# dwkim606/optimal_conv

Measured on AMD Instinct MI355X. Metric: homomorphic convs/sec (conv_then_pack + BN bias, k x k, batch B, N=2^16), higher is better.
Workload: dtype u64; 1 GPU; conv 3 3; ker_wid=3, batch=256, in_wid=16, logN=16, moduli=ckks.DefaultBootstrapParams[6] Q0,Q1 + P=0x1fffffffffe00001, ciphertexts_per_launch_set=4, contexts_per_gpu=4, chunk_nodes=512

## Files before the change

optimal_conv_amd/csrc/hc_arith.h:

```cpp
#pragma once
#include <stdint.h>

#if defined(__HIPCC__) || defined(HC_EMU)
#define HC_HD __host__ __device__ __forceinline__
#else
#define HC_HD inline
#endif

typedef uint64_t u64;
typedef unsigned int u32;
typedef unsigned __int128 u128;

HC_HD u64 hc_mulhi(u64 a, u64 b) {
#if defined(__HIP_DEVICE_COMPILE__)
    return __umul64hi(a, b);
#else
    return (u64)(((u128)a * b) >> 64);
#endif
}

HC_HD u64 hc_mul_shoup_lazy(u64 x, u64 w, u64 wp, u64 q) {
    u64 hi = hc_mulhi(x, wp);
    return x * w - hi * q;
}
HC_HD double hc_f64_mulmod(double x, double w, double wq, double q) {
#pragma clang fp contract(off)
    const double h = x * w;
    const double l = __builtin_fma(x, w, -h);
    const double k = __builtin_rint(x * wq);
    const double r = __builtin_fma(-k, q, h);
    return r + l;
}
HC_HD double hc_f64_reduce(double u, double q, double qinv) {
#pragma clang fp contract(off)
    return __builtin_fma(-__builtin_rint(u * qinv), q, u);
}
HC_HD double hc_u2d(u64 x) { return __builtin_bit_cast(double, x); }
HC_HD u64 hc_d2u(double x) { return __builtin_bit_cast(u64, x); }
HC_HD double hc_f64_from_u(u64 x) { return hc_u2d(x | 0x4330000000000000ull) - 4503599627370496.0; }
HC_HD u64 hc_f64_to_u_plus(double v, u64 base) { return (hc_d2u(v + 6755399441055744.0) & 0x000FFFFFFFFFFFFFull) + (base - 0x0008000000000000ull); }

HC_HD u64 hc_shoup_companion(u64 w, u64 q) {
    u64 r = w, quo = 0;
    for (int i = 0; i < 64; i++) {
        r <<= 1; quo <<= 1;
        if (r >= q) { r -= q; quo |= 1; }
    }
    return quo;
}
HC_HD u64 hc_csub(u64 x, u64 q) { return x >= q ? x - q : x; }

HC_HD u64 hc_mulhi_lo2(u64 x, u64 p) {
    const u32 x0 = (u32)x, x1 = (u32)(x >> 32), p0 = (u32)p, p1 = (u32)(p >> 32);
    return (u64)x1 * p1 + (((u64)x0 * p1) >> 32) + (((u64)x1 * p0) >> 32);
}
HC_HD u64 hc_opaque_uniform(u64 v) {
#if defined(__HIP_DEVICE_COMPILE__)
    u64 r;
    asm("; uniform constant kept opaque" : "=s"(r) : "0"(v));
    return r;
#else
    return v;
// ... 43 lines not shown
```

optimal_conv_amd/csrc/hc_kernels.h:

```cpp
#pragma once
#include "hc_arith.h"

#define HC_TPB 256
#ifndef HC_MIN_WAVES
#define HC_MIN_WAVES 4
#endif
#define HC_ROWS_LDS 4096
#define HC_COLS_LDS 4096

struct __attribute__((aligned(16))) HcTw { u64 w, ws; };

#define HC_SMALL_Q(q) ((q) < (1ull << 31))
template <bool B> struct HcBool { static constexpr bool value = B; };
template <int V> struct HcInt { static constexpr int value = V; };
#define HC_COUNT_DISPATCH(n, body) do { switch (n) { case 1: body(HcInt<1>{}); break; case 2: body(HcInt<2>{}); break; case 3: body(HcInt<3>{}); break; case 4: body(HcInt<4>{}); break; \
    case 5: body(HcInt<5>{}); break; case 6: body(HcInt<6>{}); break; case 7: body(HcInt<7>{}); break; case 8: body(HcInt<8>{}); break; default: break; } } while (0)
#define HC_LD(S32, rowptr, j) ((S32) ? hc_ld32(rowptr, j) : (rowptr)[j])
#define HC_ST(S32, rowptr, j, v) do { if (S32) hc_st32(rowptr, j, v); else (rowptr)[j] = (v); } while (0)
#define HC_ROW_DISPATCH(row32, body) do { if (row32) body(HcBool<true>{}); else body(HcBool<false>{}); } while (0)
__device__ __forceinline__ u64 hc_ld32(const u64 *row, size_t j) { return (u64)reinterpret_cast<const u32 *>(row)[j]; }
__device__ __forceinline__ void hc_st32(u64 *row, size_t j, u64 v) { reinterpret_cast<u32 *>(row)[j] = (u32)v; }
struct __attribute__((packed, aligned(4))) HcU64A4 { u64 v; };
__device__ __forceinline__ u64 hc_ldp(const u64 *row, size_t j, bool row32) {
    return reinterpret_cast<const HcU64A4 *>(reinterpret_cast<const char *>(row) + (j << (row32 ? 2 : 3)))->v & (row32 ? 0xFFFFFFFFull : ~0ull);
// ... 618 lines not shown
        const u64 x = t[i];
        u64 r;
        if (x > (q0 >> 1)) { r = hc_barrett64(q0 - x, q, mu); r = r ? q - r : 0; }
        else r = hc_barrett64(x, q, mu);
        if (row32) hc_st32(out, i, r); else out[i] = r;
    }
}
__global__ __launch_bounds__(HC_TPB) void hc_k_shoup_companion(const u64 *w, u64 *ws, size_t n, u64 q) {
    for (size_t i = (size_t)blockIdx.x * HC_TPB + threadIdx.x; i < n; i += (size_t)gridDim.x * HC_TPB)
        ws[i] = hc_shoup_companion(w[i], q);
}
__global__ __launch_bounds__(HC_TPB) void hc_k_lo_local(const u64 *in, u64 *out, size_t n) {
    for (size_t i = (size_t)blockIdx.x * HC_TPB + threadIdx.x; i < n; i += (size_t)gridDim.x * HC_TPB) {
        const size_t poly = i >> 16; const int R = (int)((i >> 8) & 255), C = (int)(i & 255);
        out[(poly << 16) + (size_t)(((R >> 4) * 16 + (C & 15)) * 256 + (R & 15) * 16 + (C >> 4))] = in[i];
    }
}
__global__ __launch_bounds__(HC_TPB) void hc_k_make_pairs(const u64 *w, HcTw *out, size_t n, u64 q, int lo_local_order) {
    for (size_t i = (size_t)blockIdx.x * HC_TPB + threadIdx.x; i < n; i += (size_t)gridDim.x * HC_TPB) {
        u64 x = w[i];
        HcTw p; p.w = x; p.ws = hc_shoup_companion(x, q);
        size_t j = i;
        if (lo_local_order) {
            size_t poly = i >> 16; int R = (int)((i >> 8) & 255), C = (int)(i & 255);
            j = (poly << 16) + (size_t)(((R >> 4) * 16 + (C & 15)) * 256 + (R & 15) * 16 + (C >> 4));
        }
        out[j] = p;
    }
}

#define HC_MAXB 16
struct HcPtrs { const u64 *p[HC_MAXB]; };
struct HcCtc { HcMod m0, m1; HcTw c0, c1; };
__global__ __launch_bounds__(HC_TPB) void hc_k_ctc_pairs(HcPtrs ct_in, HcTw *out, HcCtc K) {
    const int r = blockIdx.y, l = r & 1; const HcMod m = l ? K.m1 : K.m0; const HcTw cst = l ? K.c1 : K.c0;
    const u64 *in = ct_in.p[blockIdx.z] + (size_t)r * 65536;
    HcTw *o = out + ((size_t)blockIdx.z * 4 + r) * 65536;
    for (size_t i = (size_t)blockIdx.x * HC_TPB + threadIdx.x; i < 65536; i += (size_t)gridDim.x * HC_TPB) {
        HcTw p; p.w = hc_mul_shoup(in[i], cst.w, cst.ws, m.q); p.ws = hc_shoup_companion(p.w, m.q);
        o[i] = p;
    }
}

struct HcPrepKer {
    const double *ker_in;
    const double *bn_a;
    u64 *stage;
    int in_wid, ker_wid, real_ib, real_ob, norm, max_bat;
    double scale;
    u64 q0, q1;
    int src_wid, dil, ib_stride;
};
__device__ __forceinline__ void hc_prep_ker_put(const HcPrepKer &P, int k_sz, int vec_size, int adj, int i, int col, double v) {
    const int jj = P.max_bat - 1 - col / k_sz, kk = k_sz - 1 - col % k_sz;
    const int p0 = (P.in_wid * (kk / P.ker_wid) + kk % P.ker_wid) * P.max_bat + jj;
    const bool wrap = p0 < adj;
    const int p = wrap ? vec_size - adj + p0 : p0 - adj;
    const double val = wrap ? -v : v;
    const bool neg = val < 0;
    const double x = neg ? -P.scale * val : P.scale * val;
    const u64 xi = (u64)(x + 0.5);
    const u64 r0 = xi % P.q0, r1 = xi % P.q1;
    P.stage[((size_t)0 * P.max_bat + i) * 65536 + p] = neg ? P.q0 - r0 : r0;
    P.stage[((size_t)1 * P.max_bat + i) * 65536 + p] = neg ? P.q1 - r1 : r1;
}
template <bool TRANS, bool EXP = false, bool FC = false>
__global__ __launch_bounds__(HC_TPB) void hc_k_prep_ker(HcPrepKer P) {
    static_assert(!(TRANS && EXP), "dilated / channel-strided kernels have no transposed form");
    static_assert(!FC || EXP, "the shared-matrix form is a form of the dilated scatter");
// ... 73 lines not shown
#ifndef HC_W_A3
#define HC_W_A3 3
#endif
#ifndef HC_W_B1
#define HC_W_B1 4
#endif
#ifndef HC_W_B2
#define HC_W_B2 1
#endif
#ifndef HC_W_B3
#define HC_W_B3 4
#endif
#ifndef HC_W_B4
#define HC_W_B4 1
#endif
#ifndef HC_A3_ROWS
#define HC_A3_ROWS 4
#endif
struct HcLoopA {
    const HcTw *ctc;
    HcPtrs ker;
    u64 *tmp;
    u64 *cts;
    int i0, norm;
    int slot0, slot_step;
    size_t cts_stride;
    int njobs;
    int gm;
    HcMod m0, m1;
    HcTw q1inv;
    u64 h, negh0;
};
template <int F64>
__global__ __launch_bounds__(HC_TPB, HC_W_A1) void hc_k_a1p(HcLoopA A, HcTwTab T1inv) {
    __shared__ __attribute__((aligned(16))) u64 lds[HC_ROWS_LDS];
    const int t = threadIdx.x, tid = t & 15, rloc = t >> 4, row = HC_TILE * 16 + rloc;
    const int ch = HC_JOB, i = A.i0 + ch * A.norm, z = blockIdx.z;
    const HcTw *__restrict__ c0 = A.ctc + ((size_t)z * 4 + 1) * 65536 + (size_t)HC_TILE * 4096 + t;
    const u64 *__restrict__ k = A.ker.p[z] + ((size_t)i * 2 + 1) * 65536 + (size_t)HC_TILE * 4096 + t;
    const HcQ Q = hc_q(A.m1.q);
    const HcTw wA = hc_twl_load(T1inv, HC_TILE, t);
    u64 e0[16], e1[16];
#pragma unroll
    for (int kk = 0; kk < 16; kk++) {
        const u64 kv = k[kk * 256];
        const HcTw w0 = c0[kk * 256], w1 = c0[2 * 65536 + kk * 256];
        e0[kk] = hc_shoup4(kv, w0.w, w0.ws, Q);
        e1[kk] = hc_shoup4(kv, w1.w, w1.ws, Q);
    }
    u64 *o = A.tmp + ((size_t)z * A.njobs + 2 * ch) * 65536 + (size_t)row * 256;
    hc_xchg(lds, [&](int kk) { return hc_rows_lds(kk, t); }, [&](int lo) { return hc_rows_lds(rloc, tid * 16 + lo); }, [] { __syncthreads(); }, e0, e1);
    HC_ROW_SYNC();
    if (F64) {
        const HcF64Mod m{(double)A.m1.q, 1.0 / (double)A.m1.q};
        double f0[16], f1[16];
#pragma unroll
        for (int kk = 0; kk < 16; kk++) { f0[kk] = hc_f64_reduce(hc_f64_from_u(e0[kk]), m.q, m.qinv); f1[kk] = hc_f64_reduce(hc_f64_from_u(e1[kk]), m.q, m.qinv); }
        hc_rows_inv2_f64(f0, f1, lds, T1inv, wA, row, rloc, tid, m);
#pragma unroll
        for (int hi = 0; hi < 16; hi++) { o[hi * 16 + tid] = hc_d2u(f0[hi]); o[65536 + hi * 16 + tid] = hc_d2u(f1[hi]); }
    } else {
        hc_rows_inv_twl(HcLazy<>{Q}, lds, T1inv, wA, row, rloc, tid, e0, e1);
#pragma unroll
        for (int hi = 0; hi < 16; hi++) { o[hi * 16 + tid] = e0[hi]; o[65536 + hi * 16 + tid] = e1[hi]; }
    }
}
__device__ __forceinline__ void hc_rows_inv2_f64_g(double (&f0)[16], double (&f1)[16], u64 *lds, const HcTwTab &T, const HcTw &wA, int row, int rloc, int tid, HcF64Mod m) {
    hc_gs_round2_f64(f0, f1, HcTwB<false, HcTw>{T.rowsB + row * 256 + tid}, m);
    u64 b0[16], b1[16];
#pragma unroll
    for (int i = 0; i < 16; i++) { b0[i] = hc_d2u(f0[i]); b1[i] = hc_d2u(f1[i]); }
    hc_xchg(lds, [&](int lo) { return hc_rows_lds(rloc, tid * 16 + lo); }, [&](int hi) { return hc_rows_lds(rloc, hi * 16 + tid); }, [] { HC_ROW_SYNC(); }, b0, b1);
#pragma unroll
    for (int i = 0; i < 16; i++) { f0[i] = hc_u2d(b0[i]); f1[i] = hc_u2d(b1[i]); }
    hc_gs_round2_f64(f0, f1, hc_twl_put(lds, wA, rloc, tid), m);
}
template <int FM>
__device__ __forceinline__ void hc_rows_fwd2_lin_g(u64 (&e0)[16], u64 (&e1)[16], u64 *lds, const HcTwTab &T, const HcTw &wA, int row, int rloc, int tid, int t, const HcQ &Q) {
    hc_ct_round(HcLazy<FM>{Q}, hc_twl_put(lds, wA, rloc, tid), e0, e1);
    HC_ROW_SYNC();
    hc_xchg(lds, [&](int hi) { return hc_rows_lds(rloc, hi * 16 + tid); }, [&](int lo) { return hc_rows_lds(rloc, tid * 16 + lo); }, [] { HC_ROW_SYNC(); }, e0, e1);
    hc_ct_round(HcLazy<FM>{Q}, HcTwB<false, HcTw>{T.rowsB + row * 256 + tid}, e0, e1);
    HC_ROW_SYNC();
    hc_xchg(lds, [&](int lo) { return hc_rows_lds(rloc, tid * 16 + lo); }, [&](int kk) { return hc_rows_lds(kk, t); }, [] { __syncthreads(); }, e0, e1);
}
template <int F64>
__global__ __launch_bounds__(HC_TPB, HC_W_A1) void hc_k_a1g(HcLoopA A, HcTwTab T1inv) {
    __shared__ __attribute__((aligned(16))) u64 lds[HC_ROWS_LDS];
    const int t = threadIdx.x, tid = t & 15, rloc = t >> 4, row = HC_TILE * 16 + rloc;
    const int ch = HC_JOB, i = A.i0 + ch * A.norm, g = blockIdx.z, m = A.gm;
    const size_t tile = (size_t)HC_TILE * 4096 + t;
    const HcQ Q = hc_q(A.m1.q);
    const HcTw wA = hc_twl_load(T1inv, HC_TILE, t);
    const HcF64Mod fm{(double)A.m1.q, 1.0 / (double)A.m1.q};
    u64 e0[16], e1[16];
    if (F64) {
        double f0[16], f1[16];
#pragma unroll
        for (int kk = 0; kk < 16; kk++) f0[kk] = f1[kk] = 0.0;
        for (int j = 0; j < m; j += 2) {
            const bool two = j + 1 < m;
            const int za = g * m + j, zb = two ? za + 1 : za;
            const HcTw *__restrict__ ca = A.ctc + ((size_t)za * 4 + 1) * 65536 + tile, *__restrict__ cb = A.ctc + ((size_t)zb * 4 + 1) * 65536 + tile;
            const u64 *__restrict__ ka = A.ker.p[za] + ((size_t)i * 2 + 1) * 65536 + tile, *__restrict__ kb = A.ker.p[zb] + ((size_t)i * 2 + 1) * 65536 + tile;
#pragma unroll
            for (int kk = 0; kk < 16; kk++) {
                const u64 kv = ka[kk * 256];
                const HcTw w0 = ca[kk * 256], w1 = ca[2 * 65536 + kk * 256];
                u64 s0 = hc_shoup4(kv, w0.w, w0.ws, Q), s1 = hc_shoup4(kv, w1.w, w1.ws, Q);
                if (two) {
                    const u64 kv2 = kb[kk * 256];
                    const HcTw x0 = cb[kk * 256], x1 = cb[2 * 65536 + kk * 256];
                    s0 += hc_shoup4(kv2, x0.w, x0.ws, Q); s1 += hc_shoup4(kv2, x1.w, x1.ws, Q);
                }
                f0[kk] += hc_f64_reduce(hc_f64_from_u(s0), fm.q, fm.qinv); f1[kk] += hc_f64_reduce(hc_f64_from_u(s1), fm.q, fm.qinv);
            }
        }
#pragma unroll
        for (int kk = 0; kk < 16; kk++) { e0[kk] = hc_d2u(hc_f64_reduce(f0[kk], fm.q, fm.qinv)); e1[kk] = hc_d2u(hc_f64_reduce(f1[kk], fm.q, fm.qinv)); }
    } else {
#pragma unroll
        for (int kk = 0; kk < 16; kk++) e0[kk] = e1[kk] = 0;
        for (int j = 0; j < m; j++) {
            const int z = g * m + j;
            const HcTw *__restrict__ c0 = A.ctc + ((size_t)z * 4 + 1) * 65536 + tile;
            const u64 *__restrict__ k = A.ker.p[z] + ((size_t)i * 2 + 1) * 65536 + tile;
#pragma unroll
            for (int kk = 0; kk < 16; kk++) {
                const u64 kv = k[kk * 256];
                const HcTw w0 = c0[kk * 256], w1 = c0[2 * 65536 + kk * 256];
                e0[kk] = hc_fold(e0[kk] + hc_canon4(hc_shoup4(kv, w0.w, w0.ws, Q), Q), Q.nq);
                e1[kk] = hc_fold(e1[kk] + hc_canon4(hc_shoup4(kv, w1.w, w1.ws, Q), Q), Q.nq);
            }
        }
    }
    u64 *o = A.tmp + ((size_t)g * A.njobs + 2 * ch) * 65536 + (size_t)row * 256;
    hc_xchg(lds, [&](int kk) { return hc_rows_lds(kk, t); }, [&](int lo) { return hc_rows_lds(rloc, tid * 16 + lo); }, [] { __syncthreads(); }, e0, e1);
    HC_ROW_SYNC();
    if (F64) {
        double f0[16], f1[16];
#pragma unroll
        for (int kk = 0; kk < 16; kk++) { f0[kk] = hc_u2d(e0[kk]); f1[kk] = hc_u2d(e1[kk]); }
        hc_rows_inv2_f64_g(f0, f1, lds, T1inv, wA, row, rloc, tid, fm);
#pragma unroll
        for (int hi = 0; hi < 16; hi++) { o[hi * 16 + tid] = hc_d2u(f0[hi]); o[65536 + hi * 16 + tid] = hc_d2u(f1[hi]); }
    } else {
        hc_rows_inv_twl(HcLazy<>{Q}, lds, T1inv, wA, row, rloc, tid, e0, e1);
#pragma unroll
        for (int hi = 0; hi < 16; hi++) { o[hi * 16 + tid] = e0[hi]; o[65536 + hi * 16 + tid] = e1[hi]; }
    }
}
template <int FM, int F64>
// ... 2002 lines not shown
```

optimal_conv_amd/csrc/hconv.hip:

```cpp
#ifdef HC_EMU
#include "hip_emu.h"
#else
#include <hip/hip_runtime.h>
#endif

#include <math.h>
#include <stdarg.h>
#include <stdio.h>
#include <string.h>

#include <atomic>
#include <map>
#include <utility>
#include <string>
#include <vector>

#include "../../include/hconv.h"
#include "../../include/hconv_test_hooks.h"
#include "hc_kernels.h"
#include "hc_gomath.h"
#ifndef HC_GX_LV
#define HC_GX_LV 64
#endif
#ifndef HC_GX_PW
// ... 51 lines not shown
    if (n > 1) fac.push_back(n);
    for (u64 g = 3;; g++) {
        bool ok = true;
        for (u64 f : fac) if (h_powmod(g, (q - 1) / f, q) == 1) { ok = false; break; }
        if (ok) return g;
    }
}
static u32 h_bitrev16(u32 x) { u32 r = 0; for (int i = 0; i < 16; i++) { r = (r << 1) | (x & 1); x >>= 1; } return r; }

struct HcModHost {
    HcMod m;
    u64 psi, psi_inv;
    HcTwTab fwd, inv;
    HcTwTab32 fwd32 = {nullptr, nullptr, nullptr, nullptr}, inv32 = {nullptr, nullptr, nullptr, nullptr};
    HcTwTab inv_f64;
    std::vector<void *> allocs;
};
struct HcEvk { HcTw *q_rows; HcTw *p_rows; u64 *q_mont; bool row_local; bool row256; };
struct HcSwk { u64 *rows = nullptr; int level = 0, beta = 0; };
struct HcProfRec { std::string name; hipEvent_t a, b; };
struct hc_ctx {
    int device = 0, nq = 0, np = 0;
    hipStream_t stream = nullptr;
    std::vector<HcModHost> mods;
    std::map<u64, HcEvk> evk;
    std::map<u64, HcSwk> swk;
    HcTw *idx_pairs = nullptr;
    u64 *idx_mont = nullptr;
    bool idx_mono = false;
    u64 idx_gen = 0;
    u64 *ws_cts = nullptr; size_t ws_cts_rows = 0;
    u64 *ws_cts2 = nullptr; size_t ws_cts2_rows = 0;
    HcTw *ws_ctc = nullptr; size_t ws_ctc_cts = 0;
    u64 *ws_tmp = nullptr; size_t ws_tmp_rows = 0;
    HcMod *d_mods = nullptr; HcTw *d_csts = nullptr;
    u64 *d_mono = nullptr;
    struct CacheBlk { size_t n = 0; hipEvent_t ev = nullptr; bool pending = false; };
    std::map<char *, CacheBlk> cache_blk; std::map<size_t, std::vector<void *>> cache_free;
    int async_alloc = 0;
#ifdef HC_EMU
    long small_mm_wgs = 0;
#else
    long small_mm_wgs = 1024;
#endif
    long allocs_live = 0;
    std::map<const char *, size_t> user_blk;
    HcRowMod *d_rowmods = nullptr;
    u64 *ws_mm = nullptr; size_t ws_mm_rows = 0;
    u64 *ws_accm = nullptr; size_t ws_accm_rows = 0;
    struct KsPlan { HcBasisExt *bx = nullptr, *bxdown = nullptr; HcTw *pinv = nullptr, *pmod = nullptr, *pinv_qlinv = nullptr, *yinv = nullptr, *yinv1 = nullptr; };
    std::map<int, KsPlan> ks_plan;
    std::map<int, HcTw *> rescale_plan;
    int nb = 1; size_t bs_poly = 0, bs_qp = 0;
    const void *hoist_cx = nullptr; int hoist_level = -1;
    long chunk_nodes = 64;
    hipEvent_t ev_fork = nullptr;
    HcCplx *enc_roots = nullptr; int *enc_rot_group = nullptr;
    u32 *d_flag = nullptr;
    u64 *crt_tab = nullptr; std::vector<int> crt_words;
    hipEvent_t ev_shard = nullptr;
    u64 *ws_gather = nullptr; size_t ws_gather_rows = 0;
    long small_levels = 16;
    long peer_access = 1;
    int xcd_rows = 1;
    int pack32 = 1;
    int rot_fuse = 1;
// ... 210 lines not shown
        std::vector<u64> mono(c->mods.size() * HC_MONO_WORDS);
        for (size_t i = 0; i < c->mods.size(); i++) {
            const u64 qi = c->mods[i].m.q, r = (u64)((((u128)1) << 64) % qi), psi256 = h_powmod(c->mods[i].psi, HC_MONO_LO, qi);
            u64 *t = &mono[i * HC_MONO_WORDS], w = r;
            for (int k = 0; k < HC_MONO_LO; k++) { t[k] = w; w = h_mulmod(w, c->mods[i].psi, qi); }
            w = r;
            for (int k = 0; k < HC_MONO_HI; k++) { t[HC_MONO_LO + k] = w; w = h_mulmod(w, psi256, qi); }
        }
        if (hcx_malloc(c, (void **)&c->d_mono, mono.size() * sizeof(u64)) != hipSuccess || hcx_h2d(c, c->d_mono, mono.data(), mono.size() * sizeof(u64)) != hipSuccess) {
            g_create_err = "hc_ctx_create: device table of psi powers"; hc_ctx_destroy(c); return HC_ERR_HIP; }
    }
    if (hcx_malloc(c, (void **)&c->d_rowmods, c->mods.size() * sizeof(HcRowMod)) != hipSuccess || hc_upload_rowmods(c) != HC_OK) { g_create_err = "hc_ctx_create: device table of transforms"; hc_ctx_destroy(c); return HC_ERR_HIP; }
    *out = c;
    return HC_OK;
}

extern "C" void hc_ctx_destroy(hc_ctx *c) {
    if (!c) return;
    hipError_t first = hipSuccess; const char *what = nullptr;
    auto D = [&](hipError_t e, const char *w) { if (e != hipSuccess && first == hipSuccess) { first = e; what = w; } };
    auto F = [&](void *d) { if (d) D(hipFree(d), "hipFree"); };
    D(hipSetDevice(c->device), "hipSetDevice");
    if (c->stream) D(hipStreamSynchronize(c->stream), "hipStreamSynchronize");
    for (auto &r : c->prof) { D(hipEventDestroy(r.a), "hipEventDestroy"); D(hipEventDestroy(r.b), "hipEventDestroy"); }
    for (auto &kv : c->cache_free) for (void *d : kv.second) F(d);
    for (auto &kv : c->cache_blk) if (kv.second.ev) D(hipEventDestroy(kv.second.ev), "hipEventDestroy");
    for (auto &mh : c->mods) for (void *d : mh.allocs) F(d);
    for (auto &kv : c->evk) { F(kv.second.q_rows); F(kv.second.p_rows); }
    for (auto &kv : c->swk) F(kv.second.rows);
    F(c->idx_pairs); F(c->ws_cts); F(c->ws_cts2); F(c->ws_gather);
    if (c->ev_fork) D(hipEventDestroy(c->ev_fork), "hipEventDestroy");
    if (c->ev_shard) D(hipEventDestroy(c->ev_shard), "hipEventDestroy");
    F(c->enc_roots); F(c->enc_rot_group); F(c->d_flag); F(c->crt_tab);
    F(c->ws_ctc); F(c->ws_tmp); F(c->d_mods); F(c->d_mono); F(c->d_rowmods); F(c->ws_mm); F(c->ws_accm);
    for (auto &kv : c->ks_plan) { F(kv.second.bx); F(kv.second.bxdown); F(kv.second.pinv); F(kv.second.pmod); F(kv.second.pinv_qlinv); }
    for (auto &kv : c->rescale_plan) F(kv.second);
    F(c->d_csts);
    if (c->t0) D(hipEventDestroy(c->t0), "hipEventDestroy");
    if (c->t1) D(hipEventDestroy(c->t1), "hipEventDestroy");
    if (c->stream) D(hipStreamDestroy(c->stream), "hipStreamDestroy");
    if (first != hipSuccess) { hc_fail(nullptr, HC_ERR_HIP, "hc_ctx_destroy: %s: %s", what, hipGetErrorString(first)); fprintf(stderr, "libhconv: %s\n", g_create_err.c_str()); }
    delete c;
}

extern "C" int hc_malloc(hc_ctx *c, size_t bytes, void **dptr) { HC_ENTER(c); if (!dptr) return hc_fail(c, HC_ERR_ARG, "hc_malloc: null"); HC_HIP(c, hcx_malloc(c, dptr, bytes)); c->allocs_live++; c->user_blk[(const char *)*dptr] = bytes; return HC_OK; }
extern "C" int hc_free(hc_ctx *c, void *dptr) {
    HC_ENTER(c);
    hipError_t e = hcx_free(c, dptr);
    if (e == hipErrorInvalidDevicePointer) return hc_fail(c, HC_ERR_ARG, "hc_free: %p was not allocated by this context (with cached allocations a block goes back to the context it came from)", dptr);
    HC_HIP(c, e);
    if (dptr) {
        c->allocs_live--;
        auto ub = c->user_blk.find((const char *)dptr);
        const size_t n = ub == c->user_blk.end() ? 1 : (ub->second ? ub->second : 1);
        if (c->hoist_cx && (const char *)c->hoist_cx >= (const char *)dptr && (const char *)c->hoist_cx < (const char *)dptr + n) hc_hoist_drop(c);
        if (ub != c->user_blk.end()) c->user_blk.erase(ub);
    }
    return HC_OK;
}
extern "C" int hc_upload(hc_ctx *c, void *dst, const void *src, size_t bytes) {
    HC_ENTER(c); if (!dst || !src) return hc_fail(c, HC_ERR_ARG, "hc_upload: null pointer");
    HC_HIP(c, hcx_h2d_async(c, dst, src, bytes));
    HC_HIP(c, hipStreamSynchronize(c->stream));
    return HC_OK;
}
extern "C" int hc_download(hc_ctx *c, void *dst, const void *src, size_t bytes) {
    HC_ENTER(c); if (!dst || !src) return hc_fail(c, HC_ERR_ARG, "hc_download: null pointer");
// ... 7 lines not shown
    return HC_OK;
}
extern "C" int hc_device_count(int *n) { if (!n) return HC_ERR_ARG; return hipGetDeviceCount(n) == hipSuccess ? HC_OK : HC_ERR_HIP; }
extern "C" int hc_copy_peer(hc_ctx *dst_ctx, void *dst, hc_ctx *src_ctx, const void *src, size_t bytes) {
    HC_ENTER(src_ctx);
    if (!dst_ctx || !dst || !src) return hc_fail(src_ctx, HC_ERR_ARG, "hc_copy_peer: null");
    if (!src_ctx->ev_shard) HC_HIP(src_ctx, hipEventCreateWithFlags(&src_ctx->ev_shard, hipEventDisableTiming));
    HC_HIP(src_ctx, hipEventRecord(src_ctx->ev_shard, src_ctx->stream));
    HC_ENTER(dst_ctx);
    HC_HIP(dst_ctx, hipStreamWaitEvent(dst_ctx->stream, src_ctx->ev_shard, 0));
    HC_HIP(dst_ctx, hipMemcpyPeerAsync(dst, dst_ctx->device, src, src_ctx->device, bytes, dst_ctx->stream));
    return HC_OK;
}
extern "C" int hc_sync(hc_ctx *c) { HC_ENTER(c); HC_HIP(c, hipStreamSynchronize(c->stream)); return hc_prof_flush(c); }

static int hc_check_mod(hc_ctx *c, int mod, const char *fn) {
    if (mod < 0 || mod >= c->nq + c->np) return hc_fail(c, HC_ERR_ARG, "%s: modulus index %d out of range", fn, mod);
    return HC_OK;
}
static dim3 hc_pw_grid(size_t n) { size_t b = (n + HC_TPB - 1) / HC_TPB; if (b > 4096) b = 4096; return dim3((unsigned)b); }

template <class T>
static int hc_ensure(hc_ctx *c, T *&ws, size_t &cap, size_t units, size_t unit_bytes) {
    if (cap >= units) return HC_OK;
    HC_HIP(c, hipStreamSynchronize(c->stream));
    if (ws) HC_HIP(c, hcx_free(c, ws));
    ws = nullptr; cap = 0;
    HC_HIP(c, hcx_malloc(c, (void **)&ws, units * unit_bytes));
    cap = units;
    return HC_OK;
}
static int hc_ensure_tmp(hc_ctx *c, size_t rows) { return hc_ensure(c, c->ws_tmp, c->ws_tmp_rows, rows, HC_N * sizeof(u64)); }
static int hc_ensure_cts(hc_ctx *c, size_t rows) { return hc_ensure(c, c->ws_cts, c->ws_cts_rows, rows, HC_N * sizeof(u64)); }
static int hc_ensure_ctc(hc_ctx *c, size_t nct) { return hc_ensure(c, c->ws_ctc, c->ws_ctc_cts, nct, 4 * HC_N * sizeof(HcTw)); }
static int hc_mm_claim(hc_ctx *c, size_t rows, u64 **t) {
    hc_hoist_drop(c);
    HC_TRY(hc_ensure(c, c->ws_mm, c->ws_mm_rows, rows, HC_N * sizeof(u64)));
    *t = c->ws_mm;
    return HC_OK;
}

extern "C" int hc_ntt(hc_ctx *c, int mod, const uint64_t *in, uint64_t *out, int count) {
    HC_ENTER(c); HC_TRY(hc_check_mod(c, mod, "hc_ntt"));
    if (!in || !out || count < 1) return hc_fail(c, HC_ERR_ARG, "hc_ntt: bad arguments");
    HcModHost &mh = c->mods[(size_t)mod];
    HC_TRY(hc_ensure_tmp(c, (size_t)count));
    HC_TRY(HC_LAUNCH_FM(mh.m.q, c, "cols_fwd", hc_k_cols_fwd, dim3(16, (unsigned)count), (const u64 *)in, c->ws_tmp, mh.fwd, mh.m.q));
    HC_TRY(HC_LAUNCH_FM(mh.m.q, c, "rows_fwd_canon", hc_k_rows_fwd_canon, dim3(16, (unsigned)count), (const u64 *)c->ws_tmp, (u64 *)out, mh.fwd, mh.m.q, mh.m.mu));
    return HC_OK;
}
extern "C" int hc_intt(hc_ctx *c, int mod, const uint64_t *in, uint64_t *out, int count) {
    HC_ENTER(c); HC_TRY(hc_check_mod(c, mod, "hc_intt"));
    if (!in || !out || count < 1) return hc_fail(c, HC_ERR_ARG, "hc_intt: bad arguments");
    HcModHost &mh = c->mods[(size_t)mod];
    HC_TRY(hc_ensure_tmp(c, (size_t)count));
    HC_TRY(hc_launch(c, "rows_inv", hc_k_rows_inv, dim3(16, (unsigned)count), (const u64 *)in, c->ws_tmp, mh.inv, mh.m.q));
    HC_TRY(hc_launch(c, "cols_inv_canon", hc_k_cols_inv_canon, dim3(16, (unsigned)count), (const u64 *)c->ws_tmp, (u64 *)out, mh.inv, mh.m.q));
    return HC_OK;
}
template <int OP>
static int hc_pw(hc_ctx *c, const char *fn, int mod, const uint64_t *a, const uint64_t *b, uint64_t *out, int count, HcTw cst) {
    HC_ENTER(c); HC_TRY(hc_check_mod(c, mod, fn));
    if (!a || !out || count < 1) return hc_fail(c, HC_ERR_ARG, "%s: bad arguments", fn);
    size_t n = (size_t)count * HC_N;
    return hc_launch(c, fn, hc_k_pointwise<OP>, hc_pw_grid(n), (const u64 *)a, (const u64 *)b, (u64 *)out, n, c->mods[(size_t)mod].m, cst);
}
extern "C" int hc_mul(hc_ctx *c, int mod, const uint64_t *a, const uint64_t *b, uint64_t *out, int count) { HcTw z; z.w = z.ws = 0; if (!b) return HC_ERR_ARG; return hc_pw<HC_PW_MUL>(c, "hc_mul", mod, a, b, out, count, z); }
// ... 233 lines not shown
extern "C" uint64_t hc_const_for(double constant, double q_level_f, uint64_t q, double *scale_mult) {
    double scale = 1.0;
    if (constant != 0) { double frac = constant - (double)(int64_t)constant; if (frac != 0) scale = q_level_f; }
    if (scale_mult) *scale_mult = scale;
    const bool neg = constant < 0;
    double x = (neg ? -scale * constant : scale * constant) + 0.5;
    u64 res;
    if (x < 18446744073709551616.0) res = (u64)x % q;
    else {
        int e; double mant = frexp(x, &e);
        u64 mi = (u64)ldexp(mant, 53); int sh = e - 53;
        u64 r = mi % q; for (int i = 0; i < sh; i++) { r += r; if (r >= q) r -= q; }
        res = r;
    }
    return neg ? q - res : res;
}

static dim3 hc_grid(int jobs, int z = 1) { return dim3(16, (unsigned)jobs, (unsigned)z); }
static HcPtrs hc_ptrs1(const u64 *p) { HcPtrs P; memset(&P, 0, sizeof P); P.p[0] = p; return P; }
static int hc_fill_loopA(hc_ctx *c, HcLoopA *A, const HcPtrs &kers, u64 *cts, size_t cts_stride, int norm) {
    const HcModHost &m0 = c->mods[0], &m1 = c->mods[1];
    A->ctc = c->ws_ctc; A->ker = kers; A->tmp = c->ws_tmp; A->cts = cts; A->i0 = 0; A->norm = norm; A->slot0 = 0; A->slot_step = norm;
    A->cts_stride = cts_stride;
    A->m0 = m0.m; A->m1 = m1.m;
    A->q1inv = h_pair(h_inv(m1.m.q % m0.m.q, m0.m.q), m0.m.q);
    A->h = (m1.m.q - 1) >> 1; A->negh0 = m0.m.q - (A->h % m0.m.q);
    return HC_OK;
}

static int hc_prepare_ctc(hc_ctx *c, const HcPtrs &ct_in, int n, const u64 cst[2]) {
    HC_TRY(hc_ensure_ctc(c, (size_t)n));
    HcCtc K; K.m0 = c->mods[0].m; K.m1 = c->mods[1].m;
    K.c0 = h_pair(cst[0] % K.m0.q, K.m0.q); K.c1 = h_pair(cst[1] % K.m1.q, K.m1.q);
    return hc_launch(c, "ctc", hc_k_ctc_pairs, dim3(64, 4, (unsigned)n), ct_in, c->ws_ctc, K);
}

static int hc_loopA_run_set(hc_ctx *c, const HcPtrs &kers, int n, int i_first, int i_stride, int nch, u64 *cts, size_t cts_stride, bool compact, int gm = 1, bool folded = false) {
    long chunk = (c->chunk_nodes < 1 ? 1 : c->chunk_nodes) / n; if (chunk < 1) chunk = 1;
    if (chunk > nch) chunk = nch;
    HC_TRY(hc_ensure_tmp(c, (size_t)n * (size_t)chunk * 2));
    HcLoopA A; HC_TRY(hc_fill_loopA(c, &A, kers, cts, cts_stride, folded ? 1 : i_stride));
    const HcModHost &m0 = c->mods[0], &m1 = c->mods[1];
    for (int j0 = 0; j0 < nch; j0 += (int)chunk) {
        const int nj = (int)((nch - j0) < chunk ? (nch - j0) : chunk);
        A.i0 = folded ? j0 : i_first + j0 * i_stride;
        A.slot0 = compact ? j0 : i_first + j0 * i_stride; A.slot_step = compact ? 1 : i_stride;
        A.njobs = 2 * nj; A.gm = gm;
        const dim3 pair = hc_grid(nj, n), flat = hc_grid(2 * nj * n);
        if (gm > 1) {
            const bool f64 = hc_f64_ok(m1.m.q);
            const HcTwTab &t1 = f64 ? m1.inv_f64 : m1.inv;
            HC_TRY(f64 ? hc_launch(c, "a1g_mulsum_rowsinv", hc_k_a1g<1>, pair, A, t1) : hc_launch(c, "a1g_mulsum_rowsinv", hc_k_a1g<0>, pair, A, t1));
            if (f64) HC_TRY(hc_fm_free(m0.m.q) ? hc_launch(c, "a2_colsinv_lift_colsfwd", hc_k_a2<HC_FM_FREE, 1>, flat, A, t1, m0.fwd) : hc_launch(c, "a2_colsinv_lift_colsfwd", hc_k_a2<HC_FM_ALT, 1>, flat, A, t1, m0.fwd));
            else HC_TRY(hc_fm_free(m0.m.q) ? hc_launch(c, "a2_colsinv_lift_colsfwd", hc_k_a2<HC_FM_FREE, 0>, flat, A, t1, m0.fwd) : hc_launch(c, "a2_colsinv_lift_colsfwd", hc_k_a2<HC_FM_ALT, 0>, flat, A, t1, m0.fwd));
            HC_TRY(HC_LAUNCH_FM(m0.m.q, c, "a3g_rowsfwd_sum_rescale", hc_k_a3g, pair, A, m0.fwd));
            continue;
        }
        if (hc_f64_ok(m1.m.q)) {
            HC_TRY(hc_launch(c, "a1_mul_rowsinv", hc_k_a1p<1>, pair, A, m1.inv_f64));
            HC_TRY(hc_fm_free(m0.m.q) ? hc_launch(c, "a2_colsinv_lift_colsfwd", hc_k_a2<HC_FM_FREE, 1>, flat, A, m1.inv_f64, m0.fwd)
                                      : hc_launch(c, "a2_colsinv_lift_colsfwd", hc_k_a2<HC_FM_ALT, 1>, flat, A, m1.inv_f64, m0.fwd));
        } else {
            HC_TRY(hc_launch(c, "a1_mul_rowsinv", hc_k_a1p<0>, pair, A, m1.inv));
            HC_TRY(hc_fm_free(m0.m.q) ? hc_launch(c, "a2_colsinv_lift_colsfwd", hc_k_a2<HC_FM_FREE, 0>, flat, A, m1.inv, m0.fwd)
                                      : hc_launch(c, "a2_colsinv_lift_colsfwd", hc_k_a2<HC_FM_ALT, 0>, flat, A, m1.inv, m0.fwd));
        }
        HC_TRY(HC_LAUNCH_FM(m0.m.q, c, "a3_rowsfwd_rescale", hc_k_a3p, pair, A, m0.fwd));
    }
    return HC_OK;
}
static int hc_loopA_run(hc_ctx *c, const u64 *ker, int max_ob, int norm, u64 *cts) {
    return hc_loopA_run_set(c, hc_ptrs1(ker), 1, 0, norm, max_ob / norm, cts, 0, false);
}

static int hc_rescale_plan(hc_ctx *c, int level, const HcTw **out) {
    auto it = c->rescale_plan.find(level);
    if (it == c->rescale_plan.end()) {
        const u64 qL = c->mods[(size_t)level].m.q;
        std::vector<HcTw> h((size_t)level);
        for (int i = 0; i < level; i++) { const u64 q = c->mods[(size_t)i].m.q; h[(size_t)i] = h_pair(h_inv(qL % q, q), q); }
        HcTw *d = nullptr; HC_HIP(c, hcx_malloc(c, (void **)&d, h.size() * sizeof(HcTw)));
        HC_HIP(c, hcx_h2d(c, d, h.data(), h.size() * sizeof(HcTw)));
        it = c->rescale_plan.emplace(level, d).first;
    }
    *out = it->second;
    return HC_OK;
}
static int hc_div_round_last_n(hc_ctx *c, int level, const u64 *x, size_t xs, u64 *out, size_t os, int np) {
    if (level < 1 || level >= c->nq) return hc_fail(c, HC_ERR_ARG, "hc_div_round_last: level %d outside 1..%d", level, c->nq - 1);
    if (!x || !out) return hc_fail(c, HC_ERR_ARG, "hc_div_round_last: null");
    HC_TRY(hc_batch_fits(c, "hc_div_round_last", level, false));
    if (level != 1) {
        const HcTw *qlinv; HC_TRY(hc_rescale_plan(c, level, &qlinv));
        const int nb = c->nb, nz = np * nb;
        u64 *t; HC_TRY(hc_mm_claim(c, (size_t)nz * (level + 1), &t));
        HcInttCall mi; mi.rows = mi.nl = level + 1; mi.skip_hi = mi.out_first_row = level; mi.nz = np; mi.images = nb; mi.in = {x, xs, c->bs_poly, HC_ROWS_USER}; mi.out = {t, (size_t)HC_N, (size_t)np * HC_N, HC_ROWS_LIB8}; mi.tag = "rescale"; HC_TRY(hc_intt_mm(c, mi));
// ... 1149 lines not shown
    if (log_slots >= 0) return hc_decode_slots_impl(c, coeffs, count, log_slots, out);
    return HC_OK;
}
extern "C" int hc_lv_mul_sum(hc_ctx *c, int level, const uint64_t *const *cts, const uint64_t *pts, int ntaps, uint64_t *out) {
    HC_ENTER(c);
    if (!cts || !pts || !out || ntaps < 1 || ntaps > HC_MAXTAPS || level < 0 || level >= c->nq) return hc_fail(c, HC_ERR_ARG, "hc_lv_mul_sum: bad arguments (1 <= ntaps <= %d)", HC_MAXTAPS);
    if (c->pack32 == 2) return hc_fail(c, HC_ERR_UNSUPPORTED, "hc_lv_mul_sum: the baseline's tap sum reads 8-byte rows only (option pack32 = 2 is for the bootstrapping chain's contexts)");
    HcTapPtrs T; memset(&T, 0, sizeof T);
    for (int t = 0; t < ntaps; t++) { if (!cts[t]) return hc_fail(c, HC_ERR_ARG, "hc_lv_mul_sum: null ciphertext %d", t); T.ct[t] = (const u64 *)cts[t]; }
    return hc_launch(c, "lv_mul_sum", hc_k_lv_mul_sum, dim3(64, (unsigned)(level + 1), 2), T, (const u64 *)pts, ntaps, level + 1, (u64 *)out, (const HcMod *)c->d_mods);
}
extern "C" int hc_bl_post_ker_slots(hc_ctx *c, const double *max_ker_rs, int in_wid, int ker_wid, int pad, int max_batch, int rot, double *values_out) {
    HC_ENTER(c);
    if (!max_ker_rs || !values_out || in_wid < 1 || ker_wid < 1 || max_batch < 1 || (long)max_batch * in_wid * in_wid > HC_N / 2) return hc_fail(c, HC_ERR_ARG, "hc_bl_post_ker_slots: bad arguments");
    return hc_launch(c, "bl_post_ker", hc_k_bl_post_ker, dim3(128, (unsigned)(ker_wid * ker_wid)), max_ker_rs, (HcCplx *)values_out, in_wid, ker_wid, pad, max_batch, rot);
}

extern "C" int hc_row_is32(hc_ctx *c, int mod) {
    if (!c || mod < 0 || mod >= c->nq + c->np) return 0;
    return c->mods[(size_t)mod].m.row32 ? 1 : 0;
}
extern "C" int hc_set_option(hc_ctx *c, const char *name, long value) {
    if (!c || !name) return HC_ERR_ARG;
    if (!strcmp(name, "chunk_nodes")) { if (value < 1) return hc_fail(c, HC_ERR_ARG, "chunk_nodes must be >= 1"); c->chunk_nodes = value; return HC_OK; }
    if (!strcmp(name, "small_levels")) { if (value < 0) return hc_fail(c, HC_ERR_ARG, "small_levels must be >= 0"); c->small_levels = value; return HC_OK; }
    if (!strcmp(name, "peer_access")) { c->peer_access = value ? 1 : 0; return HC_OK; }
    if (!strcmp(name, "profile")) { hc_prof_flush(c); c->profile = value ? 1 : 0; return HC_OK; }
    if (!strcmp(name, "small_mm_wgs")) { if (value < 0) return hc_fail(c, HC_ERR_ARG, "small_mm_wgs must be >= 0"); c->small_mm_wgs = value; return HC_OK; }
    if (!strcmp(name, "rot_fuse")) { c->rot_fuse = value ? 1 : 0; return HC_OK; }
    if (!strcmp(name, "small32")) { HC_ENTER(c); c->small32 = value ? 1 : 0; HC_HIP(c, hipStreamSynchronize(c->stream)); return hc_upload_rowmods(c); }
    if (!strcmp(name, "async_alloc")) {
        if (value < 0 || value > 2) return hc_fail(c, HC_ERR_ARG, "async_alloc must be 0, 1 or 2");
        if ((int)value == c->async_alloc) return HC_OK;
        if (c->allocs_live || !c->evk.empty() || !c->swk.empty() || c->idx_pairs || c->ws_cts || c->ws_tmp || c->ws_mm || c->ws_ctc || !c->cache_blk.empty())
            return hc_fail(c, HC_ERR_STATE, "async_alloc: set it right after hc_ctx_create, before the context allocates");
        HC_ENTER(c); HC_HIP(c, hipStreamSynchronize(c->stream));
        hipStream_t ns = nullptr;
        HC_HIP(c, value ? hipStreamCreateWithFlags(&ns, hipStreamNonBlocking) : hipStreamCreate(&ns));
        HC_HIP(c, hipStreamDestroy(c->stream));
        c->stream = ns; c->async_alloc = (int)value;
        return HC_OK;
    }
    if (!strcmp(name, "pack32")) {
        if (value < 0 || value > 2) return hc_fail(c, HC_ERR_ARG, "pack32 must be 0, 1 or 2");
        if (((value == 0) != (c->pack32 == 0)) && !c->swk.empty()) return hc_fail(c, HC_ERR_STATE, "pack32: switching keys are already stored in the other form");
        HC_ENTER(c); HC_HIP(c, hipStreamSynchronize(c->stream));
        c->pack32 = (int)value; hc_hoist_drop(c);
        std::vector<HcMod> hm; for (auto &mh : c->mods) { mh.m.row32 = hc_row32(c->pack32, mh.m.q, hm.size(), c->mods.size()); hm.push_back(mh.m); }
        HC_HIP(c, hcx_h2d(c, c->d_mods, hm.data(), hm.size() * sizeof(HcMod)));
        return hc_upload_rowmods(c);
    }
    return hc_fail(c, HC_ERR_ARG, "unknown option %s", name);
}
extern "C" int hc_timer_start(hc_ctx *c) { HC_ENTER(c); HC_HIP(c, hipEventRecord(c->t0, c->stream)); return HC_OK; }
extern "C" int hc_timer_stop(hc_ctx *c, float *ms) {
    HC_ENTER(c); HC_HIP(c, hipEventRecord(c->t1, c->stream)); HC_HIP(c, hipEventSynchronize(c->t1));
    if (ms) HC_HIP(c, hipEventElapsedTime(ms, c->t0, c->t1));
    return HC_OK;
}
extern "C" int hc_profile_get(hc_ctx *c, const char *name, double *total_ms, long *launches) {
    HC_ENTER(c); HC_TRY(hc_prof_flush(c));
    if (!name) { c->prof_acc.clear(); return HC_OK; }
    auto it = c->prof_acc.find(name);
    if (total_ms) *total_ms = it == c->prof_acc.end() ? 0 : it->second.first;
    if (launches) *launches = it == c->prof_acc.end() ? 0 : it->second.second;
    return HC_OK;
}
// ... 9 lines not shown
```

Baseline: 866.4 conv/s.

## Store modulus-1 ciphertext rows as f64 and multiply in f64 in loop A1

```diff
diff --git a/optimal_conv_amd/csrc/hc_arith.h b/optimal_conv_amd/csrc/hc_arith.h
--- a/optimal_conv_amd/csrc/hc_arith.h
+++ b/optimal_conv_amd/csrc/hc_arith.h
@@ -28,6 +28,14 @@
     const double h = x * w;
     const double l = __builtin_fma(x, w, -h);
     const double k = __builtin_rint(x * wq);
+    const double r = __builtin_fma(-k, q, h);
+    return r + l;
+}
+HC_HD double hc_f64_mulmod_q(double x, double w, double q, double qinv) {
+#pragma clang fp contract(off)
+    const double h = x * w;
+    const double l = __builtin_fma(x, w, -h);
+    const double k = __builtin_rint(h * qinv);
     const double r = __builtin_fma(-k, q, h);
     return r + l;
 }
diff --git a/optimal_conv_amd/csrc/hc_kernels.h b/optimal_conv_amd/csrc/hc_kernels.h
--- a/optimal_conv_amd/csrc/hc_kernels.h
+++ b/optimal_conv_amd/csrc/hc_kernels.h
@@ -674,9 +674,14 @@
 #define HC_MAXB 16
 struct HcPtrs { const u64 *p[HC_MAXB]; };
 struct HcCtc { HcMod m0, m1; HcTw c0, c1; };
-__global__ __launch_bounds__(HC_TPB) void hc_k_ctc_pairs(HcPtrs ct_in, HcTw *out, HcCtc K) {
+__global__ __launch_bounds__(HC_TPB) void hc_k_ctc_pairs(HcPtrs ct_in, HcTw *out, double *out1, HcCtc K) {
     const int r = blockIdx.y, l = r & 1; const HcMod m = l ? K.m1 : K.m0; const HcTw cst = l ? K.c1 : K.c0;
     const u64 *in = ct_in.p[blockIdx.z] + (size_t)r * 65536;
+    if (l && out1) {
+        double *d = out1 + ((size_t)blockIdx.z * 2 + (r >> 1)) * 65536;
+        for (size_t i = (size_t)blockIdx.x * HC_TPB + threadIdx.x; i < 65536; i += (size_t)gridDim.x * HC_TPB) d[i] = hc_f64_from_u(hc_mul_shoup(in[i], cst.w, cst.ws, m.q));
+        return;
+    }
     HcTw *o = out + ((size_t)blockIdx.z * 4 + r) * 65536;
     for (size_t i = (size_t)blockIdx.x * HC_TPB + threadIdx.x; i < 65536; i += (size_t)gridDim.x * HC_TPB) {
         HcTw p; p.w = hc_mul_shoup(in[i], cst.w, cst.ws, m.q); p.ws = hc_shoup_companion(p.w, m.q);
@@ -816,34 +821,43 @@
     u64 h, negh0;
 };
 template <int F64>
-__global__ __launch_bounds__(HC_TPB, HC_W_A1) void hc_k_a1p(HcLoopA A, HcTwTab T1inv) {
+__global__ __launch_bounds__(HC_TPB, HC_W_A1) void hc_k_a1p(HcLoopA A, HcTwTab T1inv, const double *ctc1) {
     __shared__ __attribute__((aligned(16))) u64 lds[HC_ROWS_LDS];
     const int t = threadIdx.x, tid = t & 15, rloc = t >> 4, row = HC_TILE * 16 + rloc;
     const int ch = HC_JOB, i = A.i0 + ch * A.norm, z = blockIdx.z;
     const HcTw *__restrict__ c0 = A.ctc + ((size_t)z * 4 + 1) * 65536 + (size_t)HC_TILE * 4096 + t;
     const u64 *__restrict__ k = A.ker.p[z] + ((size_t)i * 2 + 1) * 65536 + (size_t)HC_TILE * 4096 + t;
-    const HcQ Q = hc_q(A.m1.q);
-    const HcTw wA = hc_twl_load(T1inv, HC_TILE, t);
-    u64 e0[16], e1[16];
-#pragma unroll
-    for (int kk = 0; kk < 16; kk++) {
-        const u64 kv = k[kk * 256];
-        const HcTw w0 = c0[kk * 256], w1 = c0[2 * 65536 + kk * 256];
-        e0[kk] = hc_shoup4(kv, w0.w, w0.ws, Q);
-        e1[kk] = hc_shoup4(kv, w1.w, w1.ws, Q);
-    }
-    u64 *o = A.tmp + ((size_t)z * A.njobs + 2 * ch) * 65536 + (size_t)row * 256;
-    hc_xchg(lds, [&](int kk) { return hc_rows_lds(kk, t); }, [&](int lo) { return hc_rows_lds(rloc, tid * 16 + lo); }, [] { __syncthreads(); }, e0, e1);
-    HC_ROW_SYNC();
-    if (F64) {
+    if constexpr (F64) {
+        const double *__restrict__ d0 = ctc1 + (size_t)z * 2 * 65536 + (size_t)HC_TILE * 4096 + t;
+        const HcTw wA = hc_twl_load(T1inv, HC_TILE, t);
         const HcF64Mod m{(double)A.m1.q, 1.0 / (double)A.m1.q};
         double f0[16], f1[16];
 #pragma unroll
-        for (int kk = 0; kk < 16; kk++) { f0[kk] = hc_f64_reduce(hc_f64_from_u(e0[kk]), m.q, m.qinv); f1[kk] = hc_f64_reduce(hc_f64_from_u(e1[kk]), m.q, m.qinv); }
+        for (int kk = 0; kk < 16; kk++) {
+            const double kv = hc_f64_from_u(k[kk * 256]);
+            f0[kk] = hc_f64_mulmod_q(kv, d0[kk * 256], m.q, m.qinv);
+            f1[kk] = hc_f64_mulmod_q(kv, d0[65536 + kk * 256], m.q, m.qinv);
+        }
+        u64 *o = A.tmp + ((size_t)z * A.njobs + 2 * ch) * 65536 + (size_t)row * 256;
+        hc_xchg(lds, [&](int kk) { return hc_rows_lds(kk, t); }, [&](int lo) { return hc_rows_lds(rloc, tid * 16 + lo); }, [] { __syncthreads(); }, f0, f1);
+        HC_ROW_SYNC();
         hc_rows_inv2_f64(f0, f1, lds, T1inv, wA, row, rloc, tid, m);
 #pragma unroll
         for (int hi = 0; hi < 16; hi++) { o[hi * 16 + tid] = hc_d2u(f0[hi]); o[65536 + hi * 16 + tid] = hc_d2u(f1[hi]); }
     } else {
+        const HcQ Q = hc_q(A.m1.q);
+        const HcTw wA = hc_twl_load(T1inv, HC_TILE, t);
+        u64 e0[16], e1[16];
+#pragma unroll
+        for (int kk = 0; kk < 16; kk++) {
+            const u64 kv = k[kk * 256];
+            const HcTw w0 = c0[kk * 256], w1 = c0[2 * 65536 + kk * 256];
+            e0[kk] = hc_shoup4(kv, w0.w, w0.ws, Q);
+            e1[kk] = hc_shoup4(kv, w1.w, w1.ws, Q);
+        }
+        u64 *o = A.tmp + ((size_t)z * A.njobs + 2 * ch) * 65536 + (size_t)row * 256;
+        hc_xchg(lds, [&](int kk) { return hc_rows_lds(kk, t); }, [&](int lo) { return hc_rows_lds(rloc, tid * 16 + lo); }, [] { __syncthreads(); }, e0, e1);
+        HC_ROW_SYNC();
         hc_rows_inv_twl(HcLazy<>{Q}, lds, T1inv, wA, row, rloc, tid, e0, e1);
 #pragma unroll
         for (int hi = 0; hi < 16; hi++) { o[hi * 16 + tid] = e0[hi]; o[65536 + hi * 16 + tid] = e1[hi]; }
@@ -869,7 +883,7 @@
     hc_xchg(lds, [&](int lo) { return hc_rows_lds(rloc, tid * 16 + lo); }, [&](int kk) { return hc_rows_lds(kk, t); }, [] { __syncthreads(); }, e0, e1);
 }
 template <int F64>
-__global__ __launch_bounds__(HC_TPB, HC_W_A1) void hc_k_a1g(HcLoopA A, HcTwTab T1inv) {
+__global__ __launch_bounds__(HC_TPB, HC_W_A1) void hc_k_a1g(HcLoopA A, HcTwTab T1inv, const double *ctc1) {
     __shared__ __attribute__((aligned(16))) u64 lds[HC_ROWS_LDS];
     const int t = threadIdx.x, tid = t & 15, rloc = t >> 4, row = HC_TILE * 16 + rloc;
     const int ch = HC_JOB, i = A.i0 + ch * A.norm, g = blockIdx.z, m = A.gm;
@@ -882,26 +896,20 @@
         double f0[16], f1[16];
 #pragma unroll
         for (int kk = 0; kk < 16; kk++) f0[kk] = f1[kk] = 0.0;
-        for (int j = 0; j < m; j += 2) {
-            const bool two = j + 1 < m;
-            const int za = g * m + j, zb = two ? za + 1 : za;
-            const HcTw *__restrict__ ca = A.ctc + ((size_t)za * 4 + 1) * 65536 + tile, *__restrict__ cb = A.ctc + ((size_t)zb * 4 + 1) * 65536 + tile;
-            const u64 *__restrict__ ka = A.ker.p[za] + ((size_t)i * 2 + 1) * 65536 + tile, *__restrict__ kb = A.ker.p[zb] + ((size_t)i * 2 + 1) * 65536 + tile;
+        for (int j = 0; j < m; j++) {
+            const int z = g * m + j;
+            const double *__restrict__ d0 = ctc1 + (size_t)z * 2 * 65536 + tile;
+            const u64 *__restrict__ k = A.ker.p[z] + ((size_t)i * 2 + 1) * 65536 + tile;
+            const bool fold = (j & 3) == 3 || j == m - 1;
 #pragma unroll
             for (int kk = 0; kk < 16; kk++) {
-                const u64 kv = ka[kk * 256];
-                const HcTw w0 = ca[kk * 256], w1 = ca[2 * 65536 + kk * 256];
-                u64 s0 = hc_shoup4(kv, w0.w, w0.ws, Q), s1 = hc_shoup4(kv, w1.w, w1.ws, Q);
-                if (two) {
-                    const u64 kv2 = kb[kk * 256];
-                    const HcTw x0 = cb[kk * 256], x1 = cb[2 * 65536 + kk * 256];
-                    s0 += hc_shoup4(kv2, x0.w, x0.ws, Q); s1 += hc_shoup4(kv2, x1.w, x1.ws, Q);
-                }
-                f0[kk] += hc_f64_reduce(hc_f64_from_u(s0), fm.q, fm.qinv); f1[kk] += hc_f64_reduce(hc_f64_from_u(s1), fm.q, fm.qinv);
-            }
-        }
-#pragma unroll
-        for (int kk = 0; kk < 16; kk++) { e0[kk] = hc_d2u(hc_f64_reduce(f0[kk], fm.q, fm.qinv)); e1[kk] = hc_d2u(hc_f64_reduce(f1[kk], fm.q, fm.qinv)); }
+                const double kv = hc_f64_from_u(k[kk * 256]);
+                f0[kk] += hc_f64_mulmod_q(kv, d0[kk * 256], fm.q, fm.qinv); f1[kk] += hc_f64_mulmod_q(kv, d0[65536 + kk * 256], fm.q, fm.qinv);
+                if (fold) { f0[kk] = hc_f64_reduce(f0[kk], fm.q, fm.qinv); f1[kk] = hc_f64_reduce(f1[kk], fm.q, fm.qinv); }
+            }
+        }
+#pragma unroll
+        for (int kk = 0; kk < 16; kk++) { e0[kk] = hc_d2u(f0[kk]); e1[kk] = hc_d2u(f1[kk]); }
     } else {
 #pragma unroll
         for (int kk = 0; kk < 16; kk++) e0[kk] = e1[kk] = 0;
diff --git a/optimal_conv_amd/csrc/hconv.hip b/optimal_conv_amd/csrc/hconv.hip
--- a/optimal_conv_amd/csrc/hconv.hip
+++ b/optimal_conv_amd/csrc/hconv.hip
@@ -107,6 +107,7 @@
     u64 *ws_cts = nullptr; size_t ws_cts_rows = 0;
     u64 *ws_cts2 = nullptr; size_t ws_cts2_rows = 0;
     HcTw *ws_ctc = nullptr; size_t ws_ctc_cts = 0;
+    double *ws_ctc1 = nullptr; size_t ws_ctc1_cts = 0;
     u64 *ws_tmp = nullptr; size_t ws_tmp_rows = 0;
     HcMod *d_mods = nullptr; HcTw *d_csts = nullptr;
     u64 *d_mono = nullptr;
@@ -383,7 +384,7 @@
     if (c->ev_fork) D(hipEventDestroy(c->ev_fork), "hipEventDestroy");
     if (c->ev_shard) D(hipEventDestroy(c->ev_shard), "hipEventDestroy");
     F(c->enc_roots); F(c->enc_rot_group); F(c->d_flag); F(c->crt_tab);
-    F(c->ws_ctc); F(c->ws_tmp); F(c->d_mods); F(c->d_mono); F(c->d_rowmods); F(c->ws_mm); F(c->ws_accm);
+    F(c->ws_ctc); F(c->ws_ctc1); F(c->ws_tmp); F(c->d_mods); F(c->d_mono); F(c->d_rowmods); F(c->ws_mm); F(c->ws_accm);
     for (auto &kv : c->ks_plan) { F(kv.second.bx); F(kv.second.bxdown); F(kv.second.pinv); F(kv.second.pmod); F(kv.second.pinv_qlinv); }
     for (auto &kv : c->rescale_plan) F(kv.second);
     F(c->d_csts);
@@ -457,7 +458,10 @@
 }
 static int hc_ensure_tmp(hc_ctx *c, size_t rows) { return hc_ensure(c, c->ws_tmp, c->ws_tmp_rows, rows, HC_N * sizeof(u64)); }
 static int hc_ensure_cts(hc_ctx *c, size_t rows) { return hc_ensure(c, c->ws_cts, c->ws_cts_rows, rows, HC_N * sizeof(u64)); }
-static int hc_ensure_ctc(hc_ctx *c, size_t nct) { return hc_ensure(c, c->ws_ctc, c->ws_ctc_cts, nct, 4 * HC_N * sizeof(HcTw)); }
+static int hc_ensure_ctc(hc_ctx *c, size_t nct) {
+    if (hc_f64_ok(c->mods[1].m.q)) HC_TRY(hc_ensure(c, c->ws_ctc1, c->ws_ctc1_cts, nct, 2 * HC_N * sizeof(double)));
+    return hc_ensure(c, c->ws_ctc, c->ws_ctc_cts, nct, 4 * HC_N * sizeof(HcTw));
+}
 static int hc_mm_claim(hc_ctx *c, size_t rows, u64 **t) {
     hc_hoist_drop(c);
     HC_TRY(hc_ensure(c, c->ws_mm, c->ws_mm_rows, rows, HC_N * sizeof(u64)));
@@ -757,7 +761,7 @@
     HC_TRY(hc_ensure_ctc(c, (size_t)n));
     HcCtc K; K.m0 = c->mods[0].m; K.m1 = c->mods[1].m;
     K.c0 = h_pair(cst[0] % K.m0.q, K.m0.q); K.c1 = h_pair(cst[1] % K.m1.q, K.m1.q);
-    return hc_launch(c, "ctc", hc_k_ctc_pairs, dim3(64, 4, (unsigned)n), ct_in, c->ws_ctc, K);
+    return hc_launch(c, "ctc", hc_k_ctc_pairs, dim3(64, 4, (unsigned)n), ct_in, c->ws_ctc, c->ws_ctc1, K);
 }
 
 static int hc_loopA_run_set(hc_ctx *c, const HcPtrs &kers, int n, int i_first, int i_stride, int nch, u64 *cts, size_t cts_stride, bool compact, int gm = 1, bool folded = false) {
@@ -775,18 +779,18 @@
         if (gm > 1) {
             const bool f64 = hc_f64_ok(m1.m.q);
             const HcTwTab &t1 = f64 ? m1.inv_f64 : m1.inv;
-            HC_TRY(f64 ? hc_launch(c, "a1g_mulsum_rowsinv", hc_k_a1g<1>, pair, A, t1) : hc_launch(c, "a1g_mulsum_rowsinv", hc_k_a1g<0>, pair, A, t1));
+            HC_TRY(f64 ? hc_launch(c, "a1g_mulsum_rowsinv", hc_k_a1g<1>, pair, A, t1, (const double *)c->ws_ctc1) : hc_launch(c, "a1g_mulsum_rowsinv", hc_k_a1g<0>, pair, A, t1, (const double *)c->ws_ctc1));
             if (f64) HC_TRY(hc_fm_free(m0.m.q) ? hc_launch(c, "a2_colsinv_lift_colsfwd", hc_k_a2<HC_FM_FREE, 1>, flat, A, t1, m0.fwd) : hc_launch(c, "a2_colsinv_lift_colsfwd", hc_k_a2<HC_FM_ALT, 1>, flat, A, t1, m0.fwd));
             else HC_TRY(hc_fm_free(m0.m.q) ? hc_launch(c, "a2_colsinv_lift_colsfwd", hc_k_a2<HC_FM_FREE, 0>, flat, A, t1, m0.fwd) : hc_launch(c, "a2_colsinv_lift_colsfwd", hc_k_a2<HC_FM_ALT, 0>, flat, A, t1, m0.fwd));
             HC_TRY(HC_LAUNCH_FM(m0.m.q, c, "a3g_rowsfwd_sum_rescale", hc_k_a3g, pair, A, m0.fwd));
             continue;
         }
         if (hc_f64_ok(m1.m.q)) {
-            HC_TRY(hc_launch(c, "a1_mul_rowsinv", hc_k_a1p<1>, pair, A, m1.inv_f64));
+            HC_TRY(hc_launch(c, "a1_mul_rowsinv", hc_k_a1p<1>, pair, A, m1.inv_f64, (const double *)c->ws_ctc1));
             HC_TRY(hc_fm_free(m0.m.q) ? hc_launch(c, "a2_colsinv_lift_colsfwd", hc_k_a2<HC_FM_FREE, 1>, flat, A, m1.inv_f64, m0.fwd)
                                       : hc_launch(c, "a2_colsinv_lift_colsfwd", hc_k_a2<HC_FM_ALT, 1>, flat, A, m1.inv_f64, m0.fwd));
         } else {
-            HC_TRY(hc_launch(c, "a1_mul_rowsinv", hc_k_a1p<0>, pair, A, m1.inv));
+            HC_TRY(hc_launch(c, "a1_mul_rowsinv", hc_k_a1p<0>, pair, A, m1.inv, (const double *)c->ws_ctc1));
             HC_TRY(hc_fm_free(m0.m.q) ? hc_launch(c, "a2_colsinv_lift_colsfwd", hc_k_a2<HC_FM_FREE, 0>, flat, A, m1.inv, m0.fwd)
                                       : hc_launch(c, "a2_colsinv_lift_colsfwd", hc_k_a2<HC_FM_ALT, 0>, flat, A, m1.inv, m0.fwd));
         }
@@ -2002,7 +2006,7 @@
     if (!strcmp(name, "async_alloc")) {
         if (value < 0 || value > 2) return hc_fail(c, HC_ERR_ARG, "async_alloc must be 0, 1 or 2");
         if ((int)value == c->async_alloc) return HC_OK;
-        if (c->allocs_live || !c->evk.empty() || !c->swk.empty() || c->idx_pairs || c->ws_cts || c->ws_tmp || c->ws_mm || c->ws_ctc || !c->cache_blk.empty())
+        if (c->allocs_live || !c->evk.empty() || !c->swk.empty() || c->idx_pairs || c->ws_cts || c->ws_tmp || c->ws_mm || c->ws_ctc || c->ws_ctc1 || !c->cache_blk.empty())
             return hc_fail(c, HC_ERR_STATE, "async_alloc: set it right after hc_ctx_create, before the context allocates");
         HC_ENTER(c); HC_HIP(c, hipStreamSynchronize(c->stream));
         hipStream_t ns = nullptr;
```

Result: faster. 877.1 conv/s, median of 6 (+1.2%).
